# jhong93/vpd

Measured on AMD Instinct MI355X. Metric: frame-crops/sec (VPD student train), higher is better.
Workload: dtype bf16; 1 GPU; configs[1]: Diving48-shaped synthetic crops 128x128, ResNet-34 student (5-ch RGB+flow), emb_dim 128, sum-MSE + AdamW, batch=256 per GPU; global_batch=256, parallelism=dp1

## Files before the change

### include/vpd_hip.h

```cpp
#ifndef VPD_HIP_H
#define VPD_HIP_H
#include <stddef.h>
#ifdef __cplusplus
extern "C" {
#endif

typedef struct vpd_plan vpd_plan_t;

const char* vpd_last_error(void);
int vpd_abi_version(void);
const char* vpd_elem_dtype(void);

int vpd_plan_create(const char* arch, int c_in, int img_h, int img_w, int emb_dim, int motion,
                    int max_batch, int train, vpd_plan_t** out);
#define VPD_TRAIN_EARLY_BUCKET0 2
void vpd_plan_destroy(vpd_plan_t* plan);

int vpd_plan_num_tensors(const vpd_plan_t* plan);
int vpd_plan_tensor_info(const vpd_plan_t* plan, int i, int* kind, int* is_decoder, long long* offset,
                         long long* numel, int* ndim, int dims[4]);
long long vpd_plan_param_numel(const vpd_plan_t* plan);
int vpd_plan_num_bn(const vpd_plan_t* plan);
int vpd_plan_bn_info(const vpd_plan_t* plan, int i, int* channels, long long* rm_off, long long* rv_off);
long long vpd_plan_bn_numel(const vpd_plan_t* plan);
// ... 100 lines not shown
                     const float* ep_shift, const void* res_padded_bf16, int ep_relu, int accumulate,
                     const unsigned char* acc_mask, void* stream);
int vpd_op_conv2d_bnsums(const void* x_bf16, const void* w_bf16, void* y_bf16, const void* bst_z_bf16,
                         const unsigned char* bst_mask, double* rows, int n, int xHp, int xWp, int xC, int Hs, int Ws,
                         int Kc, int Co, const int* tapset9, int accumulate, void* stream);
int vpd_op_conv2d_bnsums2(const void* x_bf16, const void* w_bf16, void* y_bf16, const void* bst_z_bf16,
                          const unsigned char* bst_mask, double* rows, const void* bst_z2_bf16, double* rows2, int n, int xHp,
                          int xWp, int xC, int Hs, int Ws, int Kc, int Co, const int* tapset9, void* stream);
int vpd_op_conv2d_dispatch(int n, int xHp, int xWp, int xC, int yHp, int yWp, int yC, int ypad, int Hs, int Ws, int osub, int oph,
                           int opw, int istr, int Kc, int Co, const int* tapset9, int accumulate, int flags, int* out12);
int vpd_op_bn_forward(const void* z_bf16, const double* rows, const float* gamma, const float* beta, float* running_mean,
                      float* running_var, float* mean, float* rstd, float* scale, float* shift, const void* res_padded_bf16,
                      void* out_padded_bf16, unsigned char* mask_bits, int n, int H, int W, int C, int relu, float momentum,
                      float eps, void* stream);
int vpd_op_bn_backward_apply(const void* dy_bf16, const void* z_bf16, const unsigned char* mask_bits, const double* rows,
                             const float* gamma, const float* mean, const float* rstd, void* dz_padded_bf16, float* dgamma,
                             float* dbeta, int n, int H, int W, int C, void* stream);
int vpd_op_stem_pool_forward(const void* z, const float* scale, const float* shift, void* out_padded, unsigned char* idx,
                             int n, int Hz, int Wz, int C, int opad, void* stream);
int vpd_op_stem_pool_backward(const void* dpool, const unsigned char* idx, const void* z, const float* mean, const float* rstd,
                              const float* scale, const float* shift, const float* gamma, const float* beta,
                              const void* pooled_padded, double* rows, float* coef, void* dz, float* dgamma, float* dbeta,
                              int n, int Hz, int Wz, int C, void* stream);
int vpd_op_bn_backward(void* dy, const void* z, const void* act_padded, const unsigned char* mask_bits, const float* mscale,
                       const float* mshift, const float* dy_pooled, double* rows, float* coef, void* sync, unsigned* err,
                       const float* gamma, const float* mean, const float* rstd, void* dz, int dzpad, float* dgamma,
                       float* dbeta, int n, int H, int W, int C, int write_g, int fused, void* stream);
int vpd_op_bn_backward_pair(void* dy, const void* act_padded, const void* zA, const float* meanA, const float* rstdA,
                            const float* gammaA, double* rowsA, void* dzA, float* dgammaA, float* dbetaA, const void* zB,
                            const float* meanB, const float* rstdB, const float* gammaB, double* rowsB, void* dzB,
                            float* dgammaB, float* dbetaB, void* sync, unsigned* err, int n, int H, int W, int C, void* stream);
int vpd_op_bn_backward_residency(int M, int C, int pair, int* out4);
int vpd_op_avgpool(const void* act_padded, int n, int H, int W, int C, int pad, float* pooled, void* stream);
int vpd_op_avgpool_bwd(const float* dpooled, int n, int H, int W, int C, void* dact, void* stream);
int vpd_op_sgemm(const float* A, const float* B, float* Y, const float* bias, int M, int N, int K, int ta, int tb, int relu,
                 void* stream);
int vpd_op_colsum(const float* A, int M, int N, float* out, void* stream);
int vpd_op_relu_mask(float* d, const float* act, long long n, void* stream);
int vpd_op_mse(const float* e, const float* t, long long n, float* de, float* loss_step, double* loss_accum, void* stream);
int vpd_op_wgrad(const void* dz_bf16, const void* x_bf16, float* dw, int n, int dzHp, int dzWp, int dzC, int dzpad,
                 int xHp, int xWp, int xC, int Hs, int Ws, int istr, int Kc, int Co, const int* tapset9,
                 float* slab, void* stream);
size_t vpd_op_wgrad_slab_bytes(void);
int vpd_op_wgrad_pair(const void* dz_bf16, const void* dz2_bf16, const void* x_bf16, float* dw, float* dw2, int n, int dzHp, int dzWp,
                      int dzC, int dzpad, int xHp, int xWp, int xC, int Hs, int Ws, int istr, int Kc, int Co, const int* tapset9,
                      float* slab, float* slab2, void* stream);
// ... 14 lines not shown
```

### vpd_amd/_lib.py

```python
import ctypes as C
import os

_HERE = os.path.dirname(os.path.abspath(__file__))
LIB_PATH = os.environ.get("VPD_LIB_PATH") or os.path.join(_HERE, "libvpdhip.so")
LIB_PATH_F16 = os.environ.get("VPD_LIB_PATH_F16") or os.path.join(_HERE, "libvpdhip_f16.so")
ABI_VERSION = 5

c_int_p = C.POINTER(C.c_int)
c_ll_p = C.POINTER(C.c_longlong)
vp = C.c_void_p

SIGNATURES = {
    "vpd_last_error": (C.c_char_p, []),
    "vpd_abi_version": (C.c_int, []),
    "vpd_elem_dtype": (C.c_char_p, []),
    "vpd_plan_create": (C.c_int, [C.c_char_p, C.c_int, C.c_int, C.c_int, C.c_int, C.c_int, C.c_int, C.c_int,
                                  C.POINTER(vp)]),
    "vpd_plan_destroy": (None, [vp]),
    "vpd_plan_num_tensors": (C.c_int, [vp]),
    "vpd_plan_tensor_info": (C.c_int, [vp, C.c_int, c_int_p, c_int_p, c_ll_p, c_ll_p, c_int_p, c_int_p]),
    "vpd_plan_param_numel": (C.c_longlong, [vp]),
    "vpd_plan_num_bn": (C.c_int, [vp]),
    "vpd_plan_bn_info": (C.c_int, [vp, C.c_int, c_int_p, c_ll_p, c_ll_p]),
    "vpd_plan_bn_numel": (C.c_longlong, [vp]),
# ... 25 lines not shown
    "vpd_plan_set_scale_state": (C.c_int, [vp, vp]),
    "vpd_plan_check_grads": (C.c_int, [vp, vp, C.c_longlong, vp, vp, vp]),
    "vpd_op_check_finite": (C.c_int, [vp, C.c_longlong, vp, vp]),
    "vpd_adamw_step_scaled": (C.c_int, [vp, vp, vp, vp, C.c_longlong, C.c_double, C.c_double, C.c_double, C.c_double,
                                        C.c_double, vp, vp]),
    "vpd_plan_adamw_step_scaled": (C.c_int, [vp, vp, vp, vp, vp, C.c_longlong, C.c_double, C.c_double, C.c_double, C.c_double,
                                             C.c_double, vp, vp, vp]),
    "vpd_scale_state_update": (C.c_int, [vp, C.c_float, C.c_float, C.c_int, vp]),
    "vpd_plan_bucket_scratch_range": (C.c_int, [vp, C.c_int, C.POINTER(C.c_longlong), C.POINTER(C.c_longlong)]),
    "vpd_plan_grads_pending": (C.c_int, [vp]),
    "vpd_plan_materialize_grads": (C.c_int, [vp, vp, vp, vp]),
    "vpd_plan_set_timing": (C.c_int, [vp, C.c_int]),
    "vpd_plan_read_timing": (C.c_int, [vp, C.POINTER(C.c_double), C.c_int]),
    "vpd_op_conv2d": (C.c_int, [vp, vp, vp, vp] + [C.c_int] * 16 + [c_int_p, C.c_int, vp]),
    "vpd_op_conv_bm": (C.c_int, [C.c_int, C.c_int]),
    "vpd_op_conv2d_ep": (C.c_int, [vp, vp, vp] + [C.c_int] * 13 + [c_int_p, vp, vp, vp, C.c_int, C.c_int, vp, vp]),
    "vpd_op_conv2d_bnsums": (C.c_int, [vp] * 6 + [C.c_int] * 8 + [c_int_p, C.c_int, vp]),
    "vpd_op_conv2d_bnsums2": (C.c_int, [vp] * 8 + [C.c_int] * 8 + [c_int_p, vp]),
    "vpd_op_conv2d_dispatch": (C.c_int, [C.c_int] * 16 + [c_int_p, C.c_int, C.c_int, c_int_p]),
    "vpd_op_bn_forward": (C.c_int, [vp] * 13 + [C.c_int] * 5 + [C.c_float, C.c_float, vp]),
    "vpd_op_bn_backward_apply": (C.c_int, [vp] * 10 + [C.c_int] * 4 + [vp]),
    "vpd_op_stem_pool_forward": (C.c_int, [vp] * 5 + [C.c_int] * 5 + [vp]),
    "vpd_op_stem_pool_backward": (C.c_int, [vp] * 15 + [C.c_int] * 4 + [vp]),
    "vpd_op_bn_backward": (C.c_int, [vp] * 15 + [C.c_int] + [vp, vp] + [C.c_int] * 6 + [vp]),
    "vpd_op_bn_backward_pair": (C.c_int, [vp] * 20 + [C.c_int] * 4 + [vp]),
    "vpd_op_bn_backward_residency": (C.c_int, [C.c_int, C.c_int, C.c_int, c_int_p]),
    "vpd_op_avgpool": (C.c_int, [vp] + [C.c_int] * 5 + [vp, vp]),
    "vpd_op_avgpool_bwd": (C.c_int, [vp] + [C.c_int] * 4 + [vp, vp]),
    "vpd_op_sgemm": (C.c_int, [vp] * 4 + [C.c_int] * 6 + [vp]),
    "vpd_op_colsum": (C.c_int, [vp, C.c_int, C.c_int, vp, vp]),
    "vpd_op_relu_mask": (C.c_int, [vp, vp, C.c_longlong, vp]),
    "vpd_op_mse": (C.c_int, [vp, vp, C.c_longlong, vp, vp, vp, vp]),
    "vpd_op_wgrad": (C.c_int, [vp, vp, vp] + [C.c_int] * 13 + [c_int_p, vp, vp]),
    "vpd_op_wgrad_slab_bytes": (C.c_size_t, []),
    "vpd_op_wgrad_pair": (C.c_int, [vp] * 5 + [C.c_int] * 13 + [c_int_p, vp, vp, vp]),
    "vpd_op_wgrad_pair_lds_bytes": (C.c_int, [C.c_int, C.c_int, C.c_int, c_ll_p]),
    "vpd_op_tr_read_probe": (C.c_int, [vp, vp, vp]),
    "vpd_op_wgrad128_table_bytes": (C.c_size_t, []),
    "vpd_op_wgrad128_slab_floats": (C.c_size_t, [C.c_int, C.c_int]),
    "vpd_op_wgrad128_group": (C.c_int, [C.c_int, vp, vp, vp, vp, c_int_p, vp, vp]),
    "vpd_op_wgrad128_schedule": (C.c_int, [C.c_int, c_int_p, C.c_int, c_int_p, c_int_p, c_int_p, C.c_int,
                                           C.POINTER(C.c_double)]),
}

_libs = {}


class VpdHipError(RuntimeError):
    pass


def lib(dtype="bf16"):
    if dtype in _libs:
        return _libs[dtype]
    if dtype not in ("bf16", "fp16"):
        raise VpdHipError("unknown element type %r (bf16 | fp16)" % (dtype,))
    path = LIB_PATH if dtype == "bf16" else LIB_PATH_F16
    name = os.path.basename(path)
    if not os.path.isfile(path):
        raise VpdHipError(
            "%s not found at %s: build it with `python -c 'import __graft_entry__ as g; g.build()'` "
            "or `make -C vpd_amd/csrc`.  vpd_amd has no PyTorch/CPU fallback." % (name, path))
    import torch
    h = C.CDLL(path)
    ab_build = "VPD_LIB_PATH" in os.environ and dtype == "bf16"
    for sym, (res, args) in SIGNATURES.items():
        try:
            fn = getattr(h, sym)
        except AttributeError as e:
            if ab_build and (sym.startswith("vpd_op_") or sym in ("vpd_elem_dtype", "vpd_plan_set_loss_scale")):
                continue
            raise VpdHipError("%s lacks symbol %s declared in include/vpd_hip.h" % (name, sym)) from e
        fn.restype = res
        fn.argtypes = args
    if h.vpd_abi_version() != ABI_VERSION and not (ab_build and os.environ.get("VPD_LIB_ALLOW_ABI") == str(h.vpd_abi_version())):
        raise VpdHipError("%s ABI version %d != expected %d" % (name, h.vpd_abi_version(), ABI_VERSION))
    if hasattr(h, "vpd_elem_dtype") and h.vpd_elem_dtype().decode() != dtype:
        raise VpdHipError("%s was built with %s elements, %s asked for" % (path, h.vpd_elem_dtype().decode(), dtype))
    _libs[dtype] = h
    return h


def check(rc, what="", dtype="bf16"):
    if rc != 0:
        msg = lib(dtype).vpd_last_error()
        raise VpdHipError("%s failed: %s" % (what or "libvpdhip call", msg.decode() if msg else "unknown error"))
```

### vpd_amd/csrc/bn.hip

```cpp
#include "common.h"
#include "kernels.h"

static __device__ __forceinline__ void ld8(float (&dst)[8], const float* src) {
    *reinterpret_cast<float4*>(dst) = *reinterpret_cast<const float4*>(src);
    *reinterpret_cast<float4*>(dst + 4) = *reinterpret_cast<const float4*>(src + 4);
}
struct Px { int b, y, x; };
static __device__ __forceinline__ Px px_decode(int m, int HW, int W) {
    Px q;
    q.b = m / HW;
    const int r = m - q.b * HW;
    q.y = r / W;
    q.x = r - q.y * W;
    return q;
}
static __device__ __forceinline__ size_t px_padded(const Px& q, int Hp, int Wp, int pad, int C, int c) {
    return ((size_t)(q.b * Hp + q.y + pad) * Wp + q.x + pad) * C + c;
}
static __device__ __forceinline__ void mask_act(float (&g)[8], const float (&a)[8]) {
#pragma unroll
    for (int j = 0; j < 8; ++j) g[j] = a[j] > 0.f ? g[j] : 0.f;
}
static __device__ __forceinline__ void mask_affine(float (&g)[8], const float (&z)[8], const float (&msc)[8], const float (&msh)[8]) {
#pragma unroll
// ... 563 lines not shown
                a2[j] += g * ((a[j] - be[j]) * ig[j]);
            }
        }
    block_sums_to_rows(a1, a2, p.partials, p.C);
}

hipError_t vpd_launch_stem_pool_bwd(const StemPoolBwdParams& p0, float count, const float* gamma, float* dgamma,
                                    float* dbeta, float* coef, bf16_t* dz, hipStream_t s) {
    StemPoolBwdParams p = p0;
    if (p.C % 8 || 256 % (p.C / 8)) return hipErrorInvalidValue;
    const int T = vpd_bn_bwd_blocks(p.M, p.C, &p.ppb);
    p.pass = 1; p.coef = coef; p.dz = dz;
    if (vpd_switches().stem_poolsums && p.pooled) {
        StemPoolBwdParams q = p;
        const int Mo = p.M / (p.Hz * p.Wz) * p.Ho * p.Wo;
        const int To = vpd_bn_bwd_blocks(Mo, p.C, &q.ppb);
        hipLaunchKernelGGL(stem_pool_bwd_sums_kernel, dim3(To), dim3(256), 0, s, q);
    } else {
        hipLaunchKernelGGL(stem_pool_bwd_kernel, dim3(T), dim3(256), 0, s, p);
    }
    hipLaunchKernelGGL(bn_bwd_finalize_kernel, dim3((p.C + 63) / 64), dim3(64), 0, s, p.partials,
                       VPD_STAT_ROWS, p.C, count,
                       gamma, p.rstd, dgamma, dbeta, coef);
    p.pass = 2;
    if (vpd_switches().stem_quad && !(p.Hz & 1) && !(p.Wz & 1) && p.Ho == p.Hz / 2 && p.Wo == p.Wz / 2) {
        const int per = 256 / (p.C / 8);
        const long items = (long)(p.M / (p.Hz * p.Wz)) * (p.Hz / 2) * (p.Wz / 2);
        long blocks = (items + per - 1) / per;
        if (blocks > 2048) blocks = 2048;
        hipLaunchKernelGGL(stem_pool_bwd_quad_kernel, dim3((unsigned)(blocks < 1 ? 1 : blocks)), dim3(256), 0, s, p, items);
    } else {
        hipLaunchKernelGGL(stem_pool_bwd_kernel, dim3(T), dim3(256), 0, s, p);
    }
    return hipGetLastError();
}

#include "sync.h"

static int vpd_bn_xcd_on() {
    return vpd_switches().bn_xcd;
}

static __device__ __forceinline__ int vpd_bn_virtual_block(int b, int grid, int R) {
    if (R <= 0 || grid != 256) return b;
    const int x = b & 7, jj = b >> 3;
    const int u = jj / R, r = jj - u * R;
    return (u * 8 + x) * R + r;
// ... 533 lines not shown
```

### vpd_amd/csrc/conv_wgrad.hip

```cpp
#include <stdio.h>
#include <stdlib.h>

#include <string.h>
#include <algorithm>
#include <utility>
#include <vector>
#include "common.h"

static __device__ __forceinline__ int wg_swz(int r, int c16) {
    const int f = ((r >> 1) & 1) | (((r >> 3) & 1) << 1);
    return r * 64 + ((((c16 >> 1) ^ f) << 4) | ((c16 & 1) << 3));
}

static __device__ __forceinline__ bf16x8 tr_frag(const bf16_t* tile, int rbase, int ctile, int lane) {
    const int g = lane >> 4, i = lane & 15, q = i >> 2, pp = i & 3;
    const int col = ctile * 16 + 4 * pp;
    const int r0 = rbase + 8 * g + q;
    const int r1 = r0 + 4;
    const int f0 = ((r0 >> 1) & 1) | (((r0 >> 3) & 1) << 1);
    const int f1 = ((r1 >> 1) & 1) | (((r1 >> 3) & 1) << 1);
    const int o0 = r0 * 64 + ((((col >> 4) ^ f0) << 4) | (col & 15));
    const int o1 = r1 * 64 + ((((col >> 4) ^ f1) << 4) | (col & 15));
    typedef s16x4 __attribute__((address_space(3))) * lds_p;
    const s16x4 lo = __builtin_amdgcn_ds_read_tr16_b64_v4i16((lds_p)(tile + o0));
    const s16x4 hi = __builtin_amdgcn_ds_read_tr16_b64_v4i16((lds_p)(tile + o1));
    s16x8 v;
    v[0] = lo[0]; v[1] = lo[1]; v[2] = lo[2]; v[3] = lo[3];
    v[4] = hi[0]; v[5] = hi[1]; v[6] = hi[2]; v[7] = hi[3];
    return __builtin_bit_cast(bf16x8, v);
}
// ... 588 lines not shown
        issue(0);
        if (nch > 1) issue(1);
        for (int c = 0; c < nch; ++c) {
            if (c + 1 < nch) asm volatile("s_waitcnt vmcnt(%0)" ::"n"(PER_CHUNK) : "memory");
            else asm volatile("s_waitcnt vmcnt(0)" ::: "memory");
            __builtin_amdgcn_s_barrier();
            if (c + 2 < nch) issue(c + 2);
        }
        return;
    }
    const int ctile = wave & 3;
    if (wave < 4) wgrad_stem_half<0, 4>(p, ring, STAGE, nch, ctile, lane);
    else wgrad_stem_half<4, 7>(p, ring, STAGE, nch, ctile, lane);
}

static bool wg_stem_eligible(const WgradParams& p, int* TR) {
    if (!(p.slab && p.xC == 8 && p.Kc == 64 && p.Co == 64 && p.istr == 2 && p.taps.nr == 7 && p.taps.nc == 1 &&
          p.taps.dy0 == 0 && p.taps.dys == 1 && p.taps.dx0 == 0 && p.taps.w0 == 0 && p.taps.wrs == 1))
        return false;
    if (p.Ws <= 0 || 64 % p.Ws != 0) return false;
    *TR = 64 / p.Ws;
    if (*TR > p.Hs || p.Hs % *TR != 0 || p.M % 64 != 0) return false;
    return ((2 * *TR + 5) * p.xWp + 7) / 8 <= 128;
}

__global__ __launch_bounds__(1024) void wgrad_slab_reduce_kernel(const float4* slab, float4* dw, long n4, int ksplit,
                                                                 int groups) {
    __shared__ float4 sh[16][64];
    const int o = threadIdx.x & 63, gi = threadIdx.x >> 6;
    const long i = (long)blockIdx.x * 64 + o;
    float4 a = {0.f, 0.f, 0.f, 0.f};
    if (i < n4)
        for (int s = gi; s < ksplit; s += groups) {
            const float4 v = slab[(long)s * n4 + i];
            a.x += v.x; a.y += v.y; a.z += v.z; a.w += v.w;
        }
    sh[gi][o] = a;
    __syncthreads();
    if (gi == 0 && i < n4) {
        for (int k = 1; k < groups; ++k) {
            const float4 v = sh[k][o];
            a.x += v.x; a.y += v.y; a.z += v.z; a.w += v.w;
        }
        dw[i] = a;
    }
}
// ... 213 lines not shown
        if (npass <= 3) VPD_LAUNCH(conv_wgrad_halo_kernel<3>, dim3(tiles, g.ksplit), dim3(768), lds, stream, p, g);
        else if (npass == 4) VPD_LAUNCH(conv_wgrad_halo_kernel<4>, dim3(tiles, g.ksplit), dim3(768), lds, stream, p, g);
        else if (npass == 5) VPD_LAUNCH(conv_wgrad_halo_kernel<5>, dim3(tiles, g.ksplit), dim3(768), lds, stream, p, g);
        else if (npass <= 10) VPD_LAUNCH((conv_wgrad_halo_kernel<10, 3>), dim3(tiles, g.ksplit), dim3(768), lds, stream, p, g);
        else VPD_LAUNCH((conv_wgrad_halo_kernel<13, 2>), dim3(tiles, g.ksplit), dim3(768), lds, stream, p, g);
        if (p.defer_reduce || VPD_ABL(p, 16)) return hipGetLastError();
        return vpd_launch_wgrad_reduce(p0, stream);
    }
    const int tiles = (p.Co / 64) * (p.Kc / 64) * p.taps.nr * p.taps.nc;
    const int nchunks = (p.M + 127) / 128;
    int ksplit = (1024 + tiles - 1) / tiles;
    if (ksplit > nchunks) ksplit = nchunks;
    if (ksplit < 1) ksplit = 1;
    int cpb = (nchunks + ksplit - 1) / ksplit;
    if (cpb < 4) cpb = nchunks < 4 ? nchunks : 4;
    ksplit = (nchunks + cpb - 1) / cpb;
    p.chunks_per_block = cpb;
    dim3 grid(tiles, ksplit);
    const size_t lds = 64 * 1024;
    VPD_LAUNCH(conv_wgrad_kernel, grid, dim3(256), lds, stream, p);
    return hipGetLastError();
}

#ifndef VPD_WG_PAIR_NS
#define VPD_WG_PAIR_NS 3
#endif
static bool wg_pair_lds(int npass, int ns, size_t* bytes) {
    const int rows = WG_CH + 32 * (npass <= 10 ? 10 : 13);
    *bytes = ((size_t)ns * rows + 2 * WG_CH) * 64 * sizeof(bf16_t);
    return ns >= 2 && npass <= 13 && *bytes <= (size_t)160 * 1024;
}
int vpd_wgrad_pair_lds_query(int H, int W, int ns, long long* bytes) {
    WgradParams p;
    memset(&p, 0, sizeof p);
    p.N = 1; p.Hs = H; p.Ws = W; p.istr = 2; p.xHp = 2 * H + 2; p.xWp = 2 * W + 2;
    WgHaloGeom g;
    if (H <= 0 || !wg_halo_geom(p, &g)) return -1;
    const int npass = (g.NHP + 31) / 32;
    size_t b = 0;
    const bool ok = wg_pair_lds(npass, ns > 0 ? ns : (npass > 10 ? 2 : VPD_WG_PAIR_NS), &b);
    if (bytes) *bytes = (long long)b;
    return ok ? 0 : 1;
}
bool vpd_wgrad_pair_ok(const WgradParams& p3, const WgradParams& p1) {
    if (!vpd_switches().wgrad_ds_ride) return false;
    WgradParams q1;
// ... 694 lines not shown
```

### vpd_amd/csrc/kernels.h

```cpp
#pragma once
#include <vector>

#include "common.h"

struct BnApplyParams {
    const bf16_t* z;
    const float* scale; const float* shift;
    int res_kind;
    const bf16_t* res; int rHp, rWp, rpad;
    const float* rscale; const float* rshift;
    bf16_t* out; int oHp, oWp, opad;
    int M, H, W, C, relu;
    unsigned char* mask_out;
    int xcd_tile_px;
};

struct StemPoolParams {
    const bf16_t* z; int Hz, Wz;
    const float* scale; const float* shift;
    bf16_t* out; int opad;
    unsigned char* idx;
    int N, Ho, Wo, C;
};

// ... 45 lines not shown

hipError_t vpd_launch_conv(const ConvParams& p, hipStream_t stream);
hipError_t vpd_launch_scale(float* x, long n, float s, hipStream_t stream);
bool vpd_conv1x1_stream_eligible(const ConvParams& p);
hipError_t vpd_launch_conv1x1_stream(const ConvParams& p, hipStream_t stream);
int vpd_conv_kernel_class(const ConvParams& p);
bool vpd_conv_takes_bn_sums(const ConvParams& p);
struct ConvDispatch {
    int kclass;
    int pws;
    int geo;
    int c64x2;
    int ws1x1, stream1x1;
    int halo;
    int bm, bn;
    int mode;
    int tiles_per_block;
};
ConvDispatch vpd_conv_dispatch(const ConvParams& p);
int vpd_conv_xcd_tile_px(const ConvParams& p);
hipError_t vpd_launch_wgrad_reduce(const WgradParams& p, hipStream_t stream);
extern "C" int vpd_conv_bm(int M, int Co);
hipError_t vpd_launch_wgrad(const WgradParams& p, hipStream_t stream);
size_t vpd_wgrad_slab_bytes();
bool vpd_wgrad_group_eligible(const WgradParams& p);
size_t vpd_wgrad_group_slab_floats(int M, int Co, int Kc, int ntaps = 9);
hipError_t vpd_launch_wgrad_group(const WgradParams* ps, int n, hipStream_t stream);
bool vpd_wgrad_overwrites(const WgradParams& p);
bool vpd_wgrad_pair_ok(const WgradParams& p3, const WgradParams& p1);
hipError_t vpd_launch_wgrad_pair(const WgradParams& p3, const WgradParams& p1, hipStream_t stream);
hipError_t vpd_launch_wgrad_pair_reduce(const WgradParams& p3, const WgradParams& p1, hipStream_t stream);
int vpd_wgrad_pair_lds_query(int H, int W, int ns, long long* bytes);
bool vpd_wgrad128_eligible(const WgradParams& p);
size_t vpd_wgrad128_table_bytes();
void* vpd_wgrad128_cache_new();
void vpd_wgrad128_cache_free(void* cache);
hipError_t vpd_launch_wgrad128_group(const WgradParams* ps, int n, void* cache, void* dev_table, hipStream_t stream);
bool vpd_wgrad_halo_shape_ok(int Hout, int Wout, int stride = 1, int Hin = 0, int Win = 0);

hipError_t vpd_launch_bn_finalize(double* partials, int T, int C, float count, const float* gamma,
                                  const float* beta, float* rm, float* rv, float momentum, float eps,
                                  float* mean, float* rstd, float* scale, float* shift, hipStream_t s);
hipError_t vpd_launch_bn_fold(const float* gamma, const float* beta, const float* rm, const float* rv, float eps,
                              float* scale, float* shift, int C, hipStream_t s);
hipError_t vpd_launch_bn_apply(const BnApplyParams& p, hipStream_t s);
hipError_t vpd_launch_stem_pool(const StemPoolParams& p, hipStream_t s);
int vpd_bn_bwd_blocks(int M, int C, int* ppb_out);
hipError_t vpd_launch_bn_bwd(const BnBwdParams& p, float count, const float* gamma, float* dgamma, float* dbeta,
                             hipStream_t s, bool reduce_done = false);
hipError_t vpd_launch_stem_pool_bwd(const StemPoolBwdParams& p, float count, const float* gamma, float* dgamma,
                                    float* dbeta, float* coef, bf16_t* dz, hipStream_t s);

struct BnFusedFwd {
    double* rows; float count; const float* gamma; const float* beta; float* rm; float* rv;
    float* mean; float* rstd; float* scale; float* shift;
    double* rows2; float count2; const float* gamma2; const float* beta2; float* rm2; float* rv2;
    float* mean2; float* rstd2; float* scale2; float* shift2;
    float momentum, eps;
};
struct BnFusedBwd {
    double* rows; void* sync; unsigned* err;
    const float* gamma; float* dgamma; float* dbeta; float count;
};
struct BnBwdSecond {
    BnFusedBwd f;
    const bf16_t* z; const float* mean; const float* rstd;
    bf16_t* dz;
};
#define VPD_GRID_SYNC_BYTES (18 * 128)
hipError_t vpd_launch_bn_fwd_fused(const BnApplyParams& p, const BnFusedFwd& f, hipStream_t s);
bool vpd_conv1x1_bn_eligible(const ConvParams& p);
bool vpd_conv1x1_bn2_eligible(const ConvParams& p);
// ... 62 lines not shown
```

### vpd_amd/csrc/plan.hip

```cpp
#include <hip/hip_runtime.h>
#include <math.h>
#include <stdio.h>
#include <stdlib.h>
#include <string.h>

#include <string>
#include <algorithm>
#include <vector>

#include "plan.h"

static thread_local std::string g_err;
int fail(const char* what, hipError_t e) {
    char buf[512];
    if (e != hipSuccess) snprintf(buf, sizeof buf, "%s: %s", what, hipGetErrorString(e));
    else snprintf(buf, sizeof buf, "%s", what);
    g_err = buf;
    return -1;
}

extern "C" const char* vpd_last_error(void) { return g_err.c_str(); }
extern "C" const char* vpd_elem_dtype(void) { return VPD_ELEM_NAME; }
extern "C" int vpd_abi_version(void) { return 5; }

// ... 851 lines not shown
    q.out = (bf16_t*)out_padded; q.opad = opad; q.idx = idx;
    q.N = n; q.Ho = (Hz - 1) / 2 + 1; q.Wo = (Wz - 1) / 2 + 1; q.C = C;
    LCHECK(vpd_launch_stem_pool(q, (hipStream_t)stream));
    return 0;
}

extern "C" int vpd_op_stem_pool_backward(const void* dpool, const unsigned char* idx, const void* z, const float* mean,
                                         const float* rstd, const float* scale, const float* shift, const float* gamma,
                                         const float* beta, const void* pooled_padded, double* rows, float* coef, void* dz,
                                         float* dgamma, float* dbeta, int n, int Hz, int Wz, int C, void* stream) {
    if (!dpool || !idx || !z || !mean || !rstd || !scale || !shift || !gamma || !beta || !rows || !coef || !dz || !dgamma || !dbeta)
        return fail("null argument");
    if (n < 1 || Hz < 1 || Wz < 1 || C < 8 || C % 8 || 256 % (C / 8)) return fail("bad shape");
    StemPoolBwdParams sb;
    memset(&sb, 0, sizeof sb);
    sb.dpool = (const bf16_t*)dpool; sb.idx = idx; sb.z = (const bf16_t*)z;
    sb.mean = mean; sb.rstd = rstd; sb.scale = scale; sb.shift = shift; sb.partials = rows;
    sb.pooled = (const bf16_t*)pooled_padded; sb.ppad = 1; sb.gamma_p = gamma; sb.beta_p = beta;
    sb.M = n * Hz * Wz; sb.Hz = Hz; sb.Wz = Wz; sb.Ho = (Hz - 1) / 2 + 1; sb.Wo = (Wz - 1) / 2 + 1; sb.C = C;
    LCHECK(vpd_launch_stem_pool_bwd(sb, (float)sb.M, gamma, dgamma, dbeta, coef, (bf16_t*)dz, (hipStream_t)stream));
    return 0;
}

static BnBwdParams op_bn_bwd_params(void* dy, const void* z, const void* act_padded, const float* mean, const float* rstd,
                                    void* dz, int dzpad, int n, int H, int W, int C) {
    BnBwdParams b;
    memset(&b, 0, sizeof b);
    b.dy = (const bf16_t*)dy; b.dy_rw = (bf16_t*)dy; b.z = (const bf16_t*)z;
    b.act = (const bf16_t*)act_padded; b.aHp = H + 2; b.aWp = W + 2; b.apad = 1;
    b.mean = mean; b.rstd = rstd;
    b.dz = (bf16_t*)dz; b.dzHp = H + 2 * dzpad; b.dzWp = W + 2 * dzpad; b.dzpad = dzpad;
    b.M = n * H * W; b.H = H; b.W = W; b.C = C;
    return b;
}

extern "C" int vpd_op_bn_backward(void* dy, const void* z, const void* act_padded, const unsigned char* mask_bits,
                                  const float* mscale, const float* mshift, const float* dy_pooled, double* rows, float* coef,
                                  void* sync, unsigned* err, const float* gamma, const float* mean, const float* rstd, void* dz,
                                  int dzpad, float* dgamma, float* dbeta, int n, int H, int W, int C, int write_g, int fused,
                                  void* stream) {
    if (!dy || !z || !rows || !gamma || !mean || !rstd || !dz || !dgamma || !dbeta) return fail("null argument");
    if (n < 1 || H < 1 || W < 1 || C < 8 || C % 8 || dzpad < 0) return fail("bad shape");
    if ((mscale == nullptr) != (mshift == nullptr)) return fail("mscale and mshift come together");
    if ((act_padded != nullptr) + (mask_bits != nullptr) + (mscale != nullptr) > 1) return fail("one ReLU mask at most");
    if (write_g && !act_padded) return fail("write_g goes with the activation mask");
    BnBwdParams b = op_bn_bwd_params(dy, z, act_padded, mean, rstd, dz, dzpad, n, H, W, C);
// ... 159 lines not shown
```

### vpd_amd/csrc/step.hip

```cpp
#include <hip/hip_runtime.h>
#include <string.h>

#include <algorithm>
#include <vector>

#include "plan.h"

namespace {

struct Ctx {
    vpd_plan* p;
    char* ws;
    hipStream_t s;
    const float* params;
    int n;
    bf16_t* b16(size_t off) const { return reinterpret_cast<bf16_t*>(ws + off); }
    float* f32(size_t off) const { return reinterpret_cast<float*>(ws + off); }
    unsigned char* u8(size_t off) const { return reinterpret_cast<unsigned char*>(ws + off); }
    bf16_t* dz(const ConvInfo& cv, size_t shared_off) const { return b16(cv.dz_own_off ? cv.dz_own_off : shared_off); }
    double* stat_rows() const { return reinterpret_cast<double*>(ws + p->partial_off); }
    double* bn_rows(const BnInfo& b) const { return reinterpret_cast<double*>(ws + b.rows_off); }
    bool fused(const ConvInfo& cv) const { return p->fused_bn && !cv.stem; }
    float* bn_mean(const BnInfo& b) const { return f32(b.fl_off); }
    float* bn_rstd(const BnInfo& b) const { return f32(b.fl_off) + b.C; }
// ... 146 lines not shown
            k.taps.dx0 = (pw + cv.pad - tf) / 2 + 1; k.taps.dxs = -1;
            k.taps.w0 = rf * cv.k + tf; k.taps.wrs = 2 * cv.k; k.taps.wcs = 2;
            if (ncls == 0) {
                q.Hs = k.geo.Hs; q.Ws = k.geo.Ws; q.M = k.geo.M; q.oph = ph; q.opw = pw; q.taps = k.taps;
            } else {
                q.cls[ncls - 1] = k;
            }
            ++ncls;
        }
    if (ncls == 0) return hipSuccess;
    q.ncls = ncls;
    if (ds) {
        if (q.oph != 0 || q.opw != 0 || q.taps.nr != 1 || q.taps.nc != 1 || ds->Co != cv.Co) return hipErrorInvalidValue;
        q.x2 = dzd; q.w2 = c.b16(c.p->arena_off) + ds->dgr_off; q.Kc2 = ds->Co;
    }
    if (sums) {
        q.bst_z = sums->z; q.bst_mask = sums->mask;
        q.stats = sums->rows; q.stat_rows = VPD_FUSED_ROWS;
        if (accumulate || !vpd_conv_takes_bn_sums(q)) return hipErrorInvalidValue;
    }
    return vpd_launch_conv(q, c.s);
}

hipError_t run_conv_wgrad(const Ctx& c, const ConvInfo& cv, const bf16_t* dz, const bf16_t* x, ZeroRanges* collect_zero = nullptr) {
    WgradParams q = wgrad_params(cv, c.n, dz, x);
    if (cv.stem) { q.dzHp = cv.Hout; q.dzWp = cv.Wout; q.dzpad = 0; q.xHp = c.p->xHp; q.xWp = c.p->xWp; q.xC = 8; }
    q.dw = c.f32(c.p->wg_off) + cv.wg_off;
    float* slab = c.f32(c.p->slab_off);
    q.slab = cv.slab_off >= 0 ? slab + cv.slab_off : (cv.stem ? slab : nullptr);
    q.prefer_halo_1x1 = !c.p->bottleneck;
    if (cv.slab_off >= 0 && !vpd_wgrad_overwrites(q)) q.slab = nullptr;
    if (collect_zero) {
        if (!vpd_wgrad_overwrites(q) && collect_zero->count < ZR_MAX) {
            collect_zero->ptr[collect_zero->count] = q.dw;
            collect_zero->n4[collect_zero->count++] = (long)cv.ntaps * cv.Co * cv.Kc / 4;
        }
        return hipSuccess;
    }
    if (vpd_wgrad_overwrites(q) && !cv.stem) {
        hipError_t e;
        {
            TimeScope ts(c.p, c.s, cv.stride == 1 ? 5 : 6, conv_flops(cv, c.n));
            q.defer_reduce = 1;
            e = vpd_launch_wgrad(q, c.s);
        }
        if (e != hipSuccess) return e;
        return vpd_launch_wgrad_reduce(q, c.s);
    }
    TimeScope ts(c.p, c.s, cv.stem ? 7 : (vpd_wgrad_overwrites(q) ? 5 : 6), conv_flops(cv, c.n));
    return vpd_launch_wgrad(q, c.s);
}

static void wgrad_pair_params(const Ctx& c, const ConvInfo& c1, const ConvInfo& cd, const bf16_t* dz1, const bf16_t* dzd, const bf16_t* x,
                              WgradParams* q3, WgradParams* q1) {
    float* slab = c.f32(c.p->slab_off);
    const ConvInfo* cvs[2] = {&c1, &cd};
    WgradParams* qs[2] = {q3, q1};
    for (int i = 0; i < 2; ++i) {
        *qs[i] = wgrad_params(*cvs[i], c.n, i ? dzd : dz1, x);
        qs[i]->dw = c.f32(c.p->wg_off) + cvs[i]->wg_off;
        qs[i]->slab = cvs[i]->slab_off >= 0 ? slab + cvs[i]->slab_off : nullptr;
        qs[i]->prefer_halo_1x1 = !c.p->bottleneck;
    }
}
bool wgrad_pair_ok(const Ctx& c, const ConvInfo& c1, const ConvInfo& cd) {
    if (c1.stem || cd.stem || c1.dz_own_off || cd.dz_own_off) return false;
    WgradParams q3, q1;
    wgrad_pair_params(c, c1, cd, c.b16(0), c.b16(0), c.b16(0), &q3, &q1);
    return vpd_wgrad_pair_ok(q3, q1);
}
hipError_t run_conv_wgrad_pair(const Ctx& c, const ConvInfo& c1, const ConvInfo& cd, const bf16_t* dz1, const bf16_t* dzd, const bf16_t* x) {
    WgradParams q3, q1;
// ... 553 lines not shown
        if (B.ds) {
            if (!bn3_pair) LCHECK(run_bn_bwd(c, B.cd, dout, nullptr, dzd, 1, 0, grads));
            LCHECK(wq.queue(B.cd, dzd, xin));
            LCHECK(run_conv_dgrad(c, B.c1, dz1, dnew, 0));
            LCHECK(run_conv_dgrad(c, B.cd, dzd, dnew, 1));
            gi = (gi + 2) % 3;
        } else {
            LCHECK(run_conv_dgrad(c, B.c1, dz1, dout, 1, nullptr, nullptr, mb3));
        }
        return wq.stage_end(bi);
    }

    int stem() {
        const vpd_plan* p = c.p;
        StemPoolBwdParams sb;
        memset(&sb, 0, sizeof sb);
        sb.dpool = G[gi]; sb.idx = c.u8(p->idx_off); sb.z = c.b16(p->z0_off);
        sb.mean = c.bn_mean(p->stem.bn); sb.rstd = c.bn_rstd(p->stem.bn);
        sb.scale = c.bn_scale(p->stem.bn); sb.shift = c.bn_shift(p->stem.bn);
        sb.g = c.b16(p->g0_off); sb.partials = c.stat_rows();
        sb.pooled = c.b16(p->p0_off); sb.ppad = 1;
        sb.gamma_p = c.params + p->stem.bn.w_off; sb.beta_p = c.params + p->stem.bn.b_off;
        sb.M = c.n * p->H0 * p->W0; sb.Hz = p->H0; sb.Wz = p->W0; sb.Ho = p->H1; sb.Wo = p->W1; sb.C = 64;
        LCHECK(vpd_launch_stem_pool_bwd(sb, (float)sb.M, c.params + p->stem.bn.w_off, grads + p->stem.bn.w_off,
                                        grads + p->stem.bn.b_off, c.bn_coef(p->stem.bn), c.b16(p->dz0_off), c.s));
        LCHECK(wq.queue(p->stem, c.b16(p->dz0_off), c.b16(p->xin_off)));
        return wq.unpack_bucket(3);
    }
};

}

extern "C" int vpd_pack_weights(vpd_plan_t* p, const float* params, const float* bn_running, void* workspace,
                                void* stream) {
    if (!p || !workspace || !params) return fail("null argument");
    if (p->bound_ws != workspace) return fail("workspace not initialised with vpd_plan_init_workspace");
    hipStream_t s = (hipStream_t)stream;
    char* ws = (char*)workspace;
    Ctx c{p, ws, s, params, 1};
    LCHECK(vpd_launch_pack_weights(reinterpret_cast<const PackDesc*>(ws + p->desc_off), (int)p->descs.size(),
                                   reinterpret_cast<const int*>(ws + p->bmap_pack_off), (int)p->bmap_pack.size() / 2,
                                   params, c.b16(p->arena_off), s));
    if (bn_running)
        for (BnInfo* b : p->bns)
            LCHECK(vpd_launch_bn_fold(params + b->w_off, params + b->b_off, bn_running + b->rm_off,
                                      bn_running + b->rv_off, kBnEps, c.bn_escale(*b), c.bn_eshift(*b), b->C, s));
    return 0;
}

// ... 130 lines not shown
```

### vpd_amd/csrc/switches.h

```cpp
#pragma once
#include <stdlib.h>

#define VPD_SWITCHES(X)                                        \
    X(fused_bn,           "VPD_FUSED_BN",          1)          \
    X(bn_pair,            "VPD_BN_PAIR",           1)          \
    X(bn_xcd,             "VPD_BN_XCD",            1)          \
    X(bn_xcd_force,       "VPD_BN_XCD_FORCE",     -1)          \
    X(dgrad_sums,         "VPD_DGRAD_SUMS",        1)          \
    X(dgrad_sums_l1,      "VPD_DGRAD_SUMS_L1",     1)          \
    X(dgrad_sums_s2,      "VPD_DGRAD_SUMS_S2",     1)          \
    X(dgrad_sums_pair,    "VPD_DGRAD_SUMS_PAIR",   1)          \
    X(dgrad_sums_1x1,     "VPD_DGRAD_SUMS_1X1",    1)          \
    X(relu_bits,          "VPD_RELU_BITS",         1)          \
    X(poolbwd_fold,       "VPD_POOLBWD_FOLD",      1)          \
    X(ds_merge,           "VPD_DS_MERGE",          1)          \
    X(pws,                "VPD_PWS",               1)          \
    X(pws_blocks,         "VPD_PWS_BLOCKS",        0)          \
    X(ws_256x64,          "VPD_WS_256x64",         1)          \
    X(ws_mw8,             "VPD_WS_MW8",            1)          \
    X(no_ws,              "VPD_NO_WS",             0)          \
    X(pws_geo,            "VPD_PWS_GEO",           1)          \
    X(pws_rot,            "VPD_PWS_ROT",           1)          \
    X(reserve_cus,        "VPD_RESERVE_CUS",       0)          \
    X(c64x2,              "VPD_C64X2",             1)          \
    X(c64_contig,         "VPD_C64_CONTIG",        1)          \
    X(conv1x1_ws,         "VPD_CONV1X1_WS",        1)          \
    X(conv_s2_ws,         "VPD_CONV_S2_WS",        1)          \
    X(conv_s2_dgrad_ws,   "VPD_CONV_S2_DGRAD_WS",  1)          \
    X(wg2,                "VPD_WG2",               1)          \
    X(wg2_1x1,            "VPD_WG2_1X1",           1)          \
    X(wg2_tco256,         "VPD_WG2_TCO256",        1)          \
    X(conv1x1_stream,     "VPD_CONV1X1_STREAM",    1)          \
    X(bneck_recompute,    "VPD_BNECK_RECOMPUTE",   1)          \
    X(wg_group,           "VPD_WG_GROUP",          1)          \
    X(wg_merge,           "VPD_WG_MERGE",          1)          \
    X(wgrad_1x1,          "VPD_WGRAD_1X1",        -1)          \
    X(wgrad_s2,           "VPD_WGRAD_S2",          1)          \
    X(wgrad_ds_ride,      "VPD_WGRAD_DS_RIDE",     1)          \
    X(stem_lds_store,     "VPD_STEM_LDS_STORE",    1)          \
    X(stem_pair,          "VPD_STEM_PAIR",         1)          \
    X(stem_quad,          "VPD_STEM_QUAD",         1)          \
    X(stem_poolsums,      "VPD_STEM_POOLSUMS",     1)          \
    X(stem_pool_fused,    "VPD_STEM_POOL_FUSED",   1)          \
    X(ablate,             "VPD_ABLATE",            0)

struct VpdSwitches {
#define VPD_SWITCH_FIELD(field, env, dflt) int field;
    VPD_SWITCHES(VPD_SWITCH_FIELD)
#undef VPD_SWITCH_FIELD
};

inline const VpdSwitches& vpd_switches() {
    static const VpdSwitches s = [] {
        VpdSwitches v;
#define VPD_SWITCH_READ(field, env, dflt) { const char* e = getenv(env); v.field = e ? atoi(e) : (dflt); }
        VPD_SWITCHES(VPD_SWITCH_READ)
#undef VPD_SWITCH_READ
        return v;
    }();
    return s;
}
```

Baseline: 77300 crops/s.

## Fuse stem pool/BN backward dz production into the stem weight-gradient kernel

Adds a fused kernel where four extra producer waves recompute the stem dz (maxpool-index routing, ReLU mask, BN backward apply) directly into the LDS ring that the wgrad waves consume, alongside the DMA of input rows. The stem pool backward now only computes statistics and coefficients, so the full-resolution dz tensor is never written to or reread from global memory. In exchange the kernel runs 768-thread blocks with hand-scheduled vmcnt waits and a more complex pipeline. It is gated by shape checks and a new switch that defaults on.

Measured after the change: 77830 crops/s, median of 6. No clear change (+0.7%).

```diff
diff --git a/include/vpd_hip.h b/include/vpd_hip.h
--- a/include/vpd_hip.h
+++ b/include/vpd_hip.h
@@ -146,6 +146,9 @@
                               const float* scale, const float* shift, const float* gamma, const float* beta,
                               const void* pooled_padded, double* rows, float* coef, void* dz, float* dgamma, float* dbeta,
                               int n, int Hz, int Wz, int C, void* stream);
+int vpd_op_stem_wgrad_fused(const void* dpool, const unsigned char* idx, const void* z, const float* mean, const float* rstd,
+                            const float* scale, const float* shift, const float* coef, const void* x_bf16, float* dw, int n,
+                            int xHp, int xWp, int Hz, int Wz, float* slab, void* dz_scratch, int* fused_out, void* stream);
 int vpd_op_bn_backward(void* dy, const void* z, const void* act_padded, const unsigned char* mask_bits, const float* mscale,
                        const float* mshift, const float* dy_pooled, double* rows, float* coef, void* sync, unsigned* err,
                        const float* gamma, const float* mean, const float* rstd, void* dz, int dzpad, float* dgamma,
diff --git a/vpd_amd/_lib.py b/vpd_amd/_lib.py
--- a/vpd_amd/_lib.py
+++ b/vpd_amd/_lib.py
@@ -71,6 +71,7 @@
     "vpd_op_bn_backward_apply": (C.c_int, [vp] * 10 + [C.c_int] * 4 + [vp]),
     "vpd_op_stem_pool_forward": (C.c_int, [vp] * 5 + [C.c_int] * 5 + [vp]),
     "vpd_op_stem_pool_backward": (C.c_int, [vp] * 15 + [C.c_int] * 4 + [vp]),
+    "vpd_op_stem_wgrad_fused": (C.c_int, [vp] * 10 + [C.c_int] * 5 + [vp, vp, c_int_p, vp]),
     "vpd_op_bn_backward": (C.c_int, [vp] * 15 + [C.c_int] + [vp, vp] + [C.c_int] * 6 + [vp]),
     "vpd_op_bn_backward_pair": (C.c_int, [vp] * 20 + [C.c_int] * 4 + [vp]),
     "vpd_op_bn_backward_residency": (C.c_int, [C.c_int, C.c_int, C.c_int, c_int_p]),
@@ -112,7 +113,7 @@
             "or `make -C vpd_amd/csrc`.  vpd_amd has no PyTorch/CPU fallback." % (name, path))
     import torch
     h = C.CDLL(path)
-    ab_build = "VPD_LIB_PATH" in os.environ and dtype == "bf16"
+    ab_build = ("VPD_LIB_PATH" if dtype == "bf16" else "VPD_LIB_PATH_F16") in os.environ
     for sym, (res, args) in SIGNATURES.items():
         try:
             fn = getattr(h, sym)
diff --git a/vpd_amd/csrc/bn.hip b/vpd_amd/csrc/bn.hip
--- a/vpd_amd/csrc/bn.hip
+++ b/vpd_amd/csrc/bn.hip
@@ -609,7 +609,15 @@
     hipLaunchKernelGGL(bn_bwd_finalize_kernel, dim3((p.C + 63) / 64), dim3(64), 0, s, p.partials,
                        VPD_STAT_ROWS, p.C, count,
                        gamma, p.rstd, dgamma, dbeta, coef);
-    p.pass = 2;
+    if (!dz) return hipGetLastError();
+    return vpd_launch_stem_pool_bwd_dz(p, coef, dz, s);
+}
+
+hipError_t vpd_launch_stem_pool_bwd_dz(const StemPoolBwdParams& p0, const float* coef, bf16_t* dz, hipStream_t s) {
+    StemPoolBwdParams p = p0;
+    if (p.C % 8 || 256 % (p.C / 8)) return hipErrorInvalidValue;
+    const int T = vpd_bn_bwd_blocks(p.M, p.C, &p.ppb);
+    p.pass = 2; p.coef = coef; p.dz = dz;
     if (vpd_switches().stem_quad && !(p.Hz & 1) && !(p.Wz & 1) && p.Ho == p.Hz / 2 && p.Wo == p.Wz / 2) {
         const int per = 256 / (p.C / 8);
         const long items = (long)(p.M / (p.Hz * p.Wz)) * (p.Hz / 2) * (p.Wz / 2);
diff --git a/vpd_amd/csrc/conv_wgrad.hip b/vpd_amd/csrc/conv_wgrad.hip
--- a/vpd_amd/csrc/conv_wgrad.hip
+++ b/vpd_amd/csrc/conv_wgrad.hip
@@ -3,9 +3,11 @@
 
 #include <string.h>
 #include <algorithm>
+#include <type_traits>
 #include <utility>
 #include <vector>
 #include "common.h"
+#include "kernels.h"
 
 static __device__ __forceinline__ int wg_swz(int r, int c16) {
     const int f = ((r >> 1) & 1) | (((r >> 3) & 1) << 1);
@@ -640,6 +642,187 @@
     *TR = 64 / p.Ws;
     if (*TR > p.Hs || p.Hs % *TR != 0 || p.M % 64 != 0) return false;
     return ((2 * *TR + 5) * p.xWp + 7) / 8 <= 128;
+}
+
+typedef __attribute__((ext_vector_type(2))) unsigned int u32x2;
+struct WgStemOperands {
+    u32x2 z[4];
+    u32x2 d[2][3];
+    unsigned iw[2][3];
+};
+static __device__ __forceinline__ void wg_gload8(u32x2& v, const void* base, unsigned byte_off) {
+    asm volatile("global_load_dwordx2 %0, %1, %2" : "+v"(v) : "v"(byte_off), "s"(base) : "memory");
+}
+static __device__ __forceinline__ void wg_gload4(unsigned& v, const void* base, unsigned byte_off) {
+    asm volatile("global_load_dword %0, %1, %2" : "+v"(v) : "v"(byte_off), "s"(base) : "memory");
+}
+template <int VMCNT>
+static __device__ __forceinline__ void wg_operands_wait(WgStemOperands& r) {
+    asm volatile("s_waitcnt vmcnt(%7)"
+                 : "+v"(r.z[0]), "+v"(r.z[1]), "+v"(r.z[2]), "+v"(r.z[3]), "+v"(r.d[0][0]), "+v"(r.d[0][1]), "+v"(r.d[0][2])
+                 : "n"(VMCNT)
+                 : "memory");
+    asm volatile(""
+                 : "+v"(r.d[1][0]), "+v"(r.d[1][1]), "+v"(r.d[1][2]), "+v"(r.iw[0][0]), "+v"(r.iw[0][1]), "+v"(r.iw[0][2]),
+                   "+v"(r.iw[1][0]), "+v"(r.iw[1][1]), "+v"(r.iw[1][2])
+                 :
+                 : "memory");
+}
+
+__global__ __launch_bounds__(768) void conv_wgrad_stem_fused_kernel(const WgradParams p, const StemPoolBwdParams sp, int TR,
+                                                                    int cpb, long xelems) {
+    constexpr int NPASS = 4, HROWS = 32 * NPASS;
+    constexpr int STAGE = (64 + HROWS) * 64;
+    constexpr int REGLOADS = 16;
+    extern __shared__ __attribute__((aligned(16))) unsigned char smem[];
+    bf16_t* ring = reinterpret_cast<bf16_t*>(smem);
+    const int tid = threadIdx.x;
+    const int lane = tid & 63;
+    const int wave = __builtin_amdgcn_readfirstlane(tid >> 6);
+    const int W0 = p.Ws, H0 = p.Hs;
+    const int nchunks_total = (p.M + 63) / 64;
+    const int chunk_begin = blockIdx.y * cpb;
+    int chunk_end = chunk_begin + cpb;
+    chunk_end = chunk_end < nchunks_total ? chunk_end : nchunks_total;
+    const int nch = chunk_end - chunk_begin;
+
+    if (wave >= 8) {
+        const int lw = wave - 8;
+        const int piece = lane & 7;
+        const int lrow = lane >> 3;
+        const int cq = lane & 15, qd = lw * 4 + (lane >> 4);
+        const int lr = (4 * qd) / W0;
+        const int kx = (4 * qd - lr * W0) >> 1;
+        const int Ho = sp.Ho, Wo = sp.Wo;
+        int ldsoff[4];
+#pragma unroll
+        for (int px = 0; px < 4; ++px) {
+            const int row = 4 * qd + px, cpc = cq >> 1;
+            ldsoff[px] = row * 64 + (((((cpc >> 1) ^ wg_f(row)) << 1) | (cpc & 1)) << 3) + (cq & 1) * 4;
+        }
+        float mu[4], rs[4], sc[4], shf[4], c1[4], c2[4], c3[4];
+#pragma unroll
+        for (int j = 0; j < 4; ++j) {
+            const int ch = cq * 4 + j;
+            mu[j] = sp.mean[ch]; rs[j] = sp.rstd[ch]; sc[j] = sp.scale[ch]; shf[j] = sp.shift[ch];
+            c1[j] = sp.coef[ch]; c2[j] = sp.coef[64 + ch]; c3[j] = sp.coef[128 + ch];
+        }
+        auto where = [&](int c, int* b, int* y) __attribute__((always_inline)) {
+            int ch = chunk_begin + c;
+            ch = ch < chunk_end - 1 ? ch : chunk_end - 1;
+            const int gr0 = ch * TR;
+            *b = gr0 / H0;
+            *y = gr0 - *b * H0 + lr;
+            return ch;
+        };
+        auto fetch = [&](int c, WgStemOperands& r) __attribute__((always_inline)) {
+            int b, y;
+            const int ch = where(c, &b, &y);
+            const unsigned zo = (((unsigned)ch * 64 + 4 * qd) * 64 + cq * 4) * (unsigned)sizeof(bf16_t);
+#pragma unroll
+            for (int px = 0; px < 4; ++px) wg_gload8(r.z[px], sp.z, zo + px * 64 * (unsigned)sizeof(bf16_t));
+            const int ky = y >> 1;
+#pragma unroll
+            for (int wy = 0; wy < 2; ++wy) {
+                const int oy = ky + wy < Ho ? ky + wy : Ho - 1;
+#pragma unroll
+                for (int wc = 0; wc < 3; ++wc) {
+                    const int ox = kx + wc < Wo ? kx + wc : Wo - 1;
+                    const unsigned po = ((unsigned)((b * Ho + oy) * Wo + ox)) * 64 + cq * 4;
+                    wg_gload8(r.d[wy][wc], sp.dpool, po * (unsigned)sizeof(bf16_t));
+                    wg_gload4(r.iw[wy][wc], sp.idx, po);
+                }
+            }
+        };
+        auto xdma = [&](int c) __attribute__((always_inline)) {
+            const int ch = chunk_begin + c;
+            bf16_t* st = ring + (c % 3) * STAGE;
+            const int gr0 = ch * TR;
+            const int b = gr0 / H0, y0 = gr0 - b * H0;
+            const long e0 = ((long)(b * p.xHp + 2 * y0) * p.xWp) * 8;
+#pragma unroll
+            for (int i = 0; i < NPASS; ++i) {
+                const int row = (lw + 4 * i) * 8 + lrow;
+                long e = e0 + (long)row * 64 + piece * 8;
+                e = e < xelems - 8 ? e : xelems - 8;
+                __builtin_amdgcn_global_load_lds((wg_gptr_t)(p.x + e), (wg_lptr_t)(st + 64 * 64 + (lw + 4 * i) * 8 * 64), 16, 0, 0);
+            }
+        };
+        auto produce = [&](int c, WgStemOperands& r, auto younger) __attribute__((always_inline)) {
+            wg_operands_wait<decltype(younger)::value>(r);
+            int b, y;
+            where(c, &b, &y);
+            const int dy = y & 1;
+            const bool y1_on = dy && (y >> 1) + 1 < Ho;
+            unsigned iw[2][3];
+#pragma unroll
+            for (int wy = 0; wy < 2; ++wy)
+#pragma unroll
+                for (int wc = 0; wc < 3; ++wc) {
+                    const bool on = (wy == 0 || y1_on) && kx + wc < Wo;
+                    iw[wy][wc] = on ? r.iw[wy][wc] : 0xffffffffu;
+                }
+            const unsigned row_tap0 = (unsigned)(dy + 1) * 3;
+            bf16_t* st = ring + (c % 3) * STAGE;
+#pragma unroll
+            for (int px = 0; px < 4; ++px) {
+                const int dx = px & 1, w0 = px >> 1;
+                u32x2 ov;
+#pragma unroll
+                for (int jj = 0; jj < 2; ++jj) {
+                    float o[2];
+#pragma unroll
+                    for (int h = 0; h < 2; ++h) {
+                        const int j = 2 * jj + h;
+                        auto elem = [&](unsigned word) __attribute__((always_inline)) {
+                            return bf2f(h ? (unsigned short)(word >> 16) : (unsigned short)(word & 0xffff));
+                        };
+                        float g = 0.f;
+#pragma unroll
+                        for (int wy = 0; wy < 2; ++wy)
+#pragma unroll
+                            for (int wx = 0; wx <= dx; ++wx) {
+                                const unsigned want = (wy ? 0u : row_tap0) + (unsigned)(dx + 1 - 2 * wx);
+                                const unsigned sel = (iw[wy][w0 + wx] >> (8 * j)) & 0xffu;
+                                g += sel == want ? elem(r.d[wy][w0 + wx][jj]) : 0.f;
+                            }
+                        const float z = elem(r.z[px][jj]);
+                        const float a = __builtin_fmaf(z, sc[j], shf[j]);
+                        g = a > 0.f ? g : 0.f;
+                        const float xh = (z - mu[j]) * rs[j];
+                        o[h] = c1[j] * __builtin_fmaf(-xh, c3[j], g - c2[j]);
+                    }
+                    ov[jj] = pack2bf(o[0], o[1]);
+                }
+                const unsigned at = (unsigned)(size_t)(wg_lptr_t)(st + ldsoff[px]);
+                asm volatile("ds_write_b64 %0, %1" ::"v"(at), "v"(ov) : "memory");
+            }
+        };
+        typedef std::integral_constant<int, REGLOADS + NPASS> after_one;
+        typedef std::integral_constant<int, 2 * NPASS + REGLOADS> after_two;
+        WgStemOperands ra = {}, rb = {};
+        fetch(0, ra);
+        fetch(1, rb);
+        xdma(0);
+        produce(0, ra, after_one());
+        fetch(2, ra);
+        if (nch > 1) { xdma(1); produce(1, rb, after_two()); }
+        fetch(3, rb);
+        auto step = [&](int c, WgStemOperands& r) __attribute__((always_inline)) {
+            if (c + 1 < nch) asm volatile("s_waitcnt vmcnt(%0) lgkmcnt(0)" ::"n"(2 * REGLOADS + NPASS) : "memory");
+            else asm volatile("s_waitcnt vmcnt(0) lgkmcnt(0)" ::: "memory");
+            __builtin_amdgcn_s_barrier();
+            if (c + 2 < nch) { xdma(c + 2); produce(c + 2, r, after_two()); fetch(c + 4, r); }
+        };
+        for (int c = 0; c < nch; c += 2) {
+            step(c, ra);
+            if (c + 1 < nch) step(c + 1, rb);
+        }
+        return;
+    }
+    const int ctile = wave & 3;
+    if (wave < 4) wgrad_stem_half<0, 4>(p, ring, STAGE, nch, ctile, lane);
+    else wgrad_stem_half<4, 7>(p, ring, STAGE, nch, ctile, lane);
 }
 
 __global__ __launch_bounds__(1024) void wgrad_slab_reduce_kernel(const float4* slab, float4* dw, long n4, int ksplit,
@@ -899,6 +1082,31 @@
     return hipGetLastError();
 }
 
+bool vpd_wgrad_stem_fused_ok(const WgradParams& p, const StemPoolBwdParams& sp) {
+    int tr;
+    if (!vpd_switches().stem_wgrad_fuse || !wg_stem_eligible(p, &tr)) return false;
+    if ((long)p.M * 64 * (long)sizeof(bf16_t) > 0xffffffffL) return false;
+    return sp.C == 64 && !(sp.Hz & 1) && !(sp.Wz & 3) && sp.Ho == sp.Hz / 2 && sp.Wo == sp.Wz / 2 && sp.Hz == p.Hs &&
+           sp.Wz == p.Ws && sp.M == p.M;
+}
+hipError_t vpd_launch_wgrad_stem_fused(const WgradParams& p, const StemPoolBwdParams& sp, hipStream_t stream) {
+    int tr_stem;
+    if (!vpd_wgrad_stem_fused_ok(p, sp) || !wg_stem_eligible(p, &tr_stem)) return hipErrorInvalidValue;
+    if (!sp.z || !sp.dpool || !sp.idx || !sp.mean || !sp.rstd || !sp.scale || !sp.shift || !sp.coef) return hipErrorInvalidValue;
+    const int nchunks = p.M / 64;
+    int ksplit = nchunks < 256 ? nchunks : 256;
+    const int cpb = (nchunks + ksplit - 1) / ksplit;
+    ksplit = (nchunks + cpb - 1) / cpb;
+    const size_t lds = (size_t)3 * (64 + 128) * 64 * sizeof(bf16_t);
+    const long xelems = (long)p.N * p.xHp * p.xWp * 8 + 64;
+    VPD_LAUNCH(conv_wgrad_stem_fused_kernel, dim3(1, ksplit), dim3(768), lds, stream, p, sp, tr_stem, cpb, xelems);
+    const long n4 = (long)7 * 64 * 64 / 4;
+    const int groups = ksplit < 16 ? ksplit : 16;
+    hipLaunchKernelGGL(wgrad_slab_reduce_kernel, dim3((unsigned)((n4 + 63) / 64)), dim3(64 * groups), 0, stream,
+                       (const float4*)p.slab, (float4*)p.dw, n4, ksplit, groups);
+    return hipGetLastError();
+}
+
 #ifndef VPD_WG_PAIR_NS
 #define VPD_WG_PAIR_NS 3
 #endif
diff --git a/vpd_amd/csrc/kernels.h b/vpd_amd/csrc/kernels.h
--- a/vpd_amd/csrc/kernels.h
+++ b/vpd_amd/csrc/kernels.h
@@ -91,6 +91,8 @@
 hipError_t vpd_launch_wgrad_reduce(const WgradParams& p, hipStream_t stream);
 extern "C" int vpd_conv_bm(int M, int Co);
 hipError_t vpd_launch_wgrad(const WgradParams& p, hipStream_t stream);
+bool vpd_wgrad_stem_fused_ok(const WgradParams& p, const StemPoolBwdParams& sp);
+hipError_t vpd_launch_wgrad_stem_fused(const WgradParams& p, const StemPoolBwdParams& sp, hipStream_t stream);
 size_t vpd_wgrad_slab_bytes();
 bool vpd_wgrad_group_eligible(const WgradParams& p);
 size_t vpd_wgrad_group_slab_floats(int M, int Co, int Kc, int ntaps = 9);
@@ -117,6 +119,7 @@
 int vpd_bn_bwd_blocks(int M, int C, int* ppb_out);
 hipError_t vpd_launch_bn_bwd(const BnBwdParams& p, float count, const float* gamma, float* dgamma, float* dbeta,
                              hipStream_t s, bool reduce_done = false);
+hipError_t vpd_launch_stem_pool_bwd_dz(const StemPoolBwdParams& p, const float* coef, bf16_t* dz, hipStream_t s);
 hipError_t vpd_launch_stem_pool_bwd(const StemPoolBwdParams& p, float count, const float* gamma, float* dgamma,
                                     float* dbeta, float* coef, bf16_t* dz, hipStream_t s);
 
diff --git a/vpd_amd/csrc/plan.hip b/vpd_amd/csrc/plan.hip
--- a/vpd_amd/csrc/plan.hip
+++ b/vpd_amd/csrc/plan.hip
@@ -897,6 +897,36 @@
     return 0;
 }
 
+extern "C" int vpd_op_stem_wgrad_fused(const void* dpool, const unsigned char* idx, const void* z, const float* mean,
+                                       const float* rstd, const float* scale, const float* shift, const float* coef,
+                                       const void* x, float* dw, int n, int xHp, int xWp, int Hz, int Wz, float* slab,
+                                       void* dz_scratch, int* fused_out, void* stream) {
+    if (!dpool || !idx || !z || !mean || !rstd || !scale || !shift || !coef || !x || !dw) return fail("null argument");
+    if (n < 1 || Hz < 1 || Wz < 1 || xHp < 2 * Hz + 5 || xWp < 2 * Wz + 6) return fail("bad shape");
+    StemPoolBwdParams sb;
+    memset(&sb, 0, sizeof sb);
+    sb.dpool = (const bf16_t*)dpool; sb.idx = idx; sb.z = (const bf16_t*)z;
+    sb.mean = mean; sb.rstd = rstd; sb.scale = scale; sb.shift = shift; sb.coef = coef;
+    sb.M = n * Hz * Wz; sb.Hz = Hz; sb.Wz = Wz; sb.Ho = (Hz - 1) / 2 + 1; sb.Wo = (Wz - 1) / 2 + 1; sb.C = 64;
+    WgradParams q;
+    memset(&q, 0, sizeof q);
+    q.dz = (const bf16_t*)dz_scratch; q.dzHp = Hz; q.dzWp = Wz; q.dzC = 64; q.dzpad = 0;
+    q.x = (const bf16_t*)x; q.xHp = xHp; q.xWp = xWp; q.xC = 8; q.dw = dw; q.slab = slab;
+    q.N = n; q.Hs = Hz; q.Ws = Wz; q.istr = 2; q.Kc = 64; q.Co = 64; q.M = sb.M;
+    q.taps.nr = 7; q.taps.nc = 1; q.taps.dy0 = 0; q.taps.dys = 1; q.taps.dx0 = 0; q.taps.dxs = 0;
+    q.taps.w0 = 0; q.taps.wrs = 1; q.taps.wcs = 0;
+    const bool fused = vpd_wgrad_stem_fused_ok(q, sb);
+    if (fused_out) *fused_out = fused ? 1 : 0;
+    if (fused) {
+        LCHECK(vpd_launch_wgrad_stem_fused(q, sb, (hipStream_t)stream));
+        return 0;
+    }
+    if (!dz_scratch) return fail("not a shape the fused stem weight gradient takes (or VPD_STEM_WGRAD_FUSE=0), and no dz scratch for the two launches");
+    LCHECK(vpd_launch_stem_pool_bwd_dz(sb, coef, (bf16_t*)dz_scratch, (hipStream_t)stream));
+    LCHECK(vpd_launch_wgrad(q, (hipStream_t)stream));
+    return 0;
+}
+
 static BnBwdParams op_bn_bwd_params(void* dy, const void* z, const void* act_padded, const float* mean, const float* rstd,
                                     void* dz, int dzpad, int n, int H, int W, int C) {
     BnBwdParams b;
diff --git a/vpd_amd/csrc/step.hip b/vpd_amd/csrc/step.hip
--- a/vpd_amd/csrc/step.hip
+++ b/vpd_amd/csrc/step.hip
@@ -192,9 +192,14 @@
     return vpd_launch_conv(q, c.s);
 }
 
-hipError_t run_conv_wgrad(const Ctx& c, const ConvInfo& cv, const bf16_t* dz, const bf16_t* x, ZeroRanges* collect_zero = nullptr) {
+static WgradParams stem_wgrad_params(const Ctx& c, const ConvInfo& cv, const bf16_t* dz, const bf16_t* x) {
     WgradParams q = wgrad_params(cv, c.n, dz, x);
-    if (cv.stem) { q.dzHp = cv.Hout; q.dzWp = cv.Wout; q.dzpad = 0; q.xHp = c.p->xHp; q.xWp = c.p->xWp; q.xC = 8; }
+    q.dzHp = cv.Hout; q.dzWp = cv.Wout; q.dzpad = 0; q.xHp = c.p->xHp; q.xWp = c.p->xWp; q.xC = 8;
+    return q;
+}
+hipError_t run_conv_wgrad(const Ctx& c, const ConvInfo& cv, const bf16_t* dz, const bf16_t* x, ZeroRanges* collect_zero = nullptr,
+                          const StemPoolBwdParams* stem_fuse = nullptr) {
+    WgradParams q = cv.stem ? stem_wgrad_params(c, cv, dz, x) : wgrad_params(cv, c.n, dz, x);
     q.dw = c.f32(c.p->wg_off) + cv.wg_off;
     float* slab = c.f32(c.p->slab_off);
     q.slab = cv.slab_off >= 0 ? slab + cv.slab_off : (cv.stem ? slab : nullptr);
@@ -218,6 +223,7 @@
         return vpd_launch_wgrad_reduce(q, c.s);
     }
     TimeScope ts(c.p, c.s, cv.stem ? 7 : (vpd_wgrad_overwrites(q) ? 5 : 6), conv_flops(cv, c.n));
+    if (stem_fuse) return vpd_launch_wgrad_stem_fused(q, *stem_fuse, c.s);
     return vpd_launch_wgrad(q, c.s);
 }
 
@@ -817,9 +823,14 @@
         sb.pooled = c.b16(p->p0_off); sb.ppad = 1;
         sb.gamma_p = c.params + p->stem.bn.w_off; sb.beta_p = c.params + p->stem.bn.b_off;
         sb.M = c.n * p->H0 * p->W0; sb.Hz = p->H0; sb.Wz = p->W0; sb.Ho = p->H1; sb.Wo = p->W1; sb.C = 64;
+        sb.coef = c.bn_coef(p->stem.bn);
+        WgradParams q = stem_wgrad_params(c, p->stem, c.b16(p->dz0_off), c.b16(p->xin_off));
+        q.slab = c.f32(p->slab_off);
+        const bool fuse = !p->stem.dz_own_off && vpd_wgrad_stem_fused_ok(q, sb);
         LCHECK(vpd_launch_stem_pool_bwd(sb, (float)sb.M, c.params + p->stem.bn.w_off, grads + p->stem.bn.w_off,
-                                        grads + p->stem.bn.b_off, c.bn_coef(p->stem.bn), c.b16(p->dz0_off), c.s));
-        LCHECK(wq.queue(p->stem, c.b16(p->dz0_off), c.b16(p->xin_off)));
+                                        grads + p->stem.bn.b_off, c.bn_coef(p->stem.bn), fuse ? nullptr : c.b16(p->dz0_off), c.s));
+        if (fuse) LCHECK(run_conv_wgrad(c, p->stem, c.b16(p->dz0_off), c.b16(p->xin_off), nullptr, &sb));
+        else LCHECK(wq.queue(p->stem, c.b16(p->dz0_off), c.b16(p->xin_off)));
         return wq.unpack_bucket(3);
     }
 };
diff --git a/vpd_amd/csrc/switches.h b/vpd_amd/csrc/switches.h
--- a/vpd_amd/csrc/switches.h
+++ b/vpd_amd/csrc/switches.h
@@ -42,6 +42,7 @@
     X(stem_quad,          "VPD_STEM_QUAD",         1)          \
     X(stem_poolsums,      "VPD_STEM_POOLSUMS",     1)          \
     X(stem_pool_fused,    "VPD_STEM_POOL_FUSED",   1)          \
+    X(stem_wgrad_fuse,    "VPD_STEM_WGRAD_FUSE",   1)          \
     X(ablate,             "VPD_ABLATE",            0)
 
 struct VpdSwitches {
```
